# I2-Multimedia-Lab/Video-Frame-Interpolation-Based-on-Deformable-Kernel-Region

Hardware: AMD Instinct MI355X
Metric: interpolated frames/sec at 1080p (hot path only: correlation + DepthFlowProjection + FilterInterpolation of DAIN_slowmotion x4) (higher is better)
Workload: dtype f32

## Files before the change

### video-frame-interpolation-based-on-deformable-kernel-region_amd/csrc/filterinterp_lds.hip

```cpp
#include "filterinterp_dev.h"
#include "filterinterp_paths.h"

namespace vfi {

#define FI_TW 64
#define FI_TH 16
#define FI_PX 2
#define FI_THREADS (FI_TW * FI_TH / FI_PX)
#define FI_PASS_ROWS (FI_TH / FI_PX)
#define FI_KS (FI_PX / 2)
#define FI_HDR 16
#define FI_RING_FLOATS 20464
#define FI_RMAX 5
#define FI_WAVES (8 / FI_PX)
#define FI_KTOP (15 * FI_KS)
static_assert(2 * FI_KTOP * FI_THREADS <= FI_RING_FLOATS, "the largest window takes two ring slots");
#define FI_B64_MIN_BH 34
#define FI_B64_MIN_BW 92
#define FI_B64_PITCH_SKEW 32

struct FiPixel {
    bool valid, inimg;
    float alpha, beta;
    int lbase;
    bool odd;
    unsigned pix;
    float f[16];
};
#define FI_BLEND_MAXC 4
struct FiBlend { const float* other; float* out; float w0, w2; };

template <int K, bool BLEND>
__device__ __forceinline__ void fi_run_channels(const float* __restrict__ img, float* __restrict__ out, int64_t cs,
                                                int c_begin, int c_end, int tid, const FiWindow& win,
                                                const FiPixel (&px)[FI_PX], float* __restrict__ ring, const FiBlend& bl) {
    constexpr int R = (FI_RING_FLOATS / (K * FI_THREADS)) < FI_RMAX ? (FI_RING_FLOATS / (K * FI_THREADS)) : FI_RMAX;
    static_assert(R >= 2 && (R - 2) * K <= 63, "vmcnt is a 6-bit counter");
    const float inv_pitch32 = 1.0f / (float)win.pitch;
    unsigned goff[K];
#pragma unroll
    for (int k = 0; k < K; ++k) {
        const int e = tid + k * FI_THREADS;
        const int r = fi_row_of(e, inv_pitch32);
        const int col = e - r * win.pitch;
        const unsigned off = 4u * (unsigned)(clampi(win.by0 + r, 0, win.h - 1) * win.hs + clampi(win.bx0 + col, 0, win.w - 1));
        goff[k] = (col < win.bw && r < win.bh) ? off : 0x80000000u;
    }
    const int plane_bytes = 4 * ((win.h - 1) * win.hs + win.w);
    constexpr int NP = K * FI_THREADS;
    constexpr int D = R - 1;
    auto issue = [&](int c, int slot) {
        const auto plane = buffer_rsrc(img + (int64_t)c * cs, plane_bytes);
        float* l = ring + slot * NP + tid;
#pragma unroll
        for (int k = 0; k < K; ++k)
            __builtin_amdgcn_raw_ptr_buffer_load_lds(plane, (lds_ptr_t)(l + k * FI_THREADS), 4, goff[k], 0, 0, 0);
    };
    auto finish = [&](int c, int p, const float (&v)[16], float* o) {
        const float val = fi4_pixel(v, px[p].f, px[p].alpha, px[p].beta);
        o[px[p].pix] = val;
        if constexpr (BLEND) {
            const float* bi = bl.other + (int64_t)c * cs;
            const float q0 = bi[px[p].pix] * bl.w0, q2 = val * bl.w2;
            float* bo = bl.out + (int64_t)c * cs;
            bo[px[p].pix] = q0 + q2;
        }
    };
    auto compute = [&](int c, int slot) {
        float* o = out + (int64_t)c * cs;
        const float* base = ring + slot * NP;
        {
#pragma unroll
            for (int p = 0; p < FI_PX; ++p) {
                if (px[p].valid) {
                    const float* t = base + px[p].lbase;
                    float v[16];
#pragma unroll
                    for (int r = 0; r < 4; ++r)
#pragma unroll
                        for (int k = 0; k < 4; ++k) v[r * 4 + k] = t[r * win.pitch + k];
                    finish(c, p, v, o);
                }
            }
        }
    };

    if (c_begin >= c_end) return;
    const int last = c_end - 1;
    for (int j = 0; j < D; ++j)
        if (c_begin + j <= last) issue(c_begin + j, j);
    wait_windows<K>(min(c_begin + D - 1, last) - c_begin);
    __builtin_amdgcn_s_barrier();
    int slot = 0;
    for (int c = c_begin; c <= last; ++c) {
        if (c + D <= last) issue(c + D, slot == 0 ? R - 1 : slot - 1);
        compute(c, slot);
        if (c < last) wait_windows<K>(min(c + D, last) - (c + 1));
        __builtin_amdgcn_s_barrier();
        slot = (slot + 1 == R) ? 0 : slot + 1;
    }
#pragma unroll
    for (int p = 0; p < FI_PX; ++p)
        if (px[p].inimg && !px[p].valid)
            for (int c = c_begin; c < c_end; ++c) {
                const float val = img[(int64_t)c * cs + px[p].pix];
                out[(int64_t)c * cs + px[p].pix] = val;
                if constexpr (BLEND) {
                    const float q0 = bl.other[(int64_t)c * cs + px[p].pix] * bl.w0, q2 = val * bl.w2;
                    bl.out[(int64_t)c * cs + px[p].pix] = q0 + q2;
                }
            }
}

template <int K, bool B64, bool DMA16 = false>
__device__ __forceinline__ void fi_run_channels_lean(const float* __restrict__ img, float* __restrict__ out, int64_t cs,
                                                     int c_begin, int c_end, int tid, const FiWindow& win,
                                                     const FiPixel (&px)[FI_PX], float* __restrict__ ring) {
    typedef float v2f __attribute__((ext_vector_type(2)));
    constexpr int EPT = DMA16 ? 4 : 1;
    constexpr int NP = K * FI_THREADS * EPT;
    constexpr int R = (FI_RING_FLOATS / NP) < FI_RMAX ? (FI_RING_FLOATS / NP) : FI_RMAX;
    constexpr int D = R - 1;
    static_assert(D >= 1 && (D - 1) * K <= 63, "ring geometry");
    static_assert((FI_HDR * 4) % 8 == 0 && (NP * 4) % 8 == 0 && FI_B64_PITCH_SKEW % 2 == 0, "8-byte tap reads stay 8-byte aligned");
    if (c_begin >= c_end) return;
    const float inv_pitch32 = 1.0f / (float)win.pitch;
    unsigned goff[K];
#pragma unroll
    for (int k = 0; k < K; ++k) {
        const int e = (tid + k * FI_THREADS) * EPT;
        const int r = fi_row_of(e, inv_pitch32);
        const int col = e - r * win.pitch;
        const unsigned off = 4u * (unsigned)(clampi(win.by0 + r, 0, win.h - 1) * win.hs + (DMA16 ? win.bx0 + col : clampi(win.bx0 + col, 0, win.w - 1)));
        goff[k] = (col < win.bw && r < win.bh) ? off : 0x80000000u;
    }
    const int plane_bytes = 4 * ((win.h - 1) * win.hs + win.w);
    const int wave_first = __builtin_amdgcn_readfirstlane(tid >> 6) * 64;
    const unsigned ring_lds = (unsigned)(uintptr_t)(lds_ptr_t)ring;
    const unsigned pitch4 = 4u * (unsigned)win.pitch;
    unsigned lb[FI_PX], soff[FI_PX];
#pragma unroll
    for (int p = 0; p < FI_PX; ++p) {
        lb[p] = ring_lds + 4u * (unsigned)px[p].lbase;
        soff[p] = px[p].valid ? 4u * px[p].pix : 0x80000000u;
    }
    v2f F[FI_PX][8];
#pragma unroll
    for (int p = 0; p < FI_PX; ++p)
#pragma unroll
        for (int r = 0; r < 4; ++r) {
            F[p][2 * r] = v2f{px[p].f[4 * r], px[p].f[4 * r + 2]};
            F[p][2 * r + 1] = v2f{px[p].f[4 * r + 1], px[p].f[4 * r + 3]};
        }
    const int last = c_end - 1;
    const float* pdma = img + (int64_t)c_begin * cs;
    float* pout = out + (int64_t)c_begin * cs;
    constexpr bool ONE = DMA16;
    auto din = buffer_rsrc(pdma, 0x7fffffff);
    auto dout = buffer_rsrc(pout, 0x7fffffff);
    const int cs4 = (int)(cs * 4);
    const int soff_max = 0x7fffffff - plane_bytes - cs4;
    int sin = 0, sout = 0;
    auto next_in = [&]() {
        if (__builtin_expect(sin > soff_max, 0)) {
            asm volatile("; the input descriptor moves up" ::: "memory");
            pdma = (const float*)((const char*)pdma + sin);
            din = buffer_rsrc(pdma, 0x7fffffff);
            sin = 0;
        }
        sin += cs4;
    };
    auto next_out = [&]() {
        if (__builtin_expect(sout > soff_max, 0)) {
            asm volatile("; the output descriptor moves up" ::: "memory");
            pout = (float*)((char*)pout + sout);
            dout = buffer_rsrc(pout, 0x7fffffff);
            sout = 0;
        }
        sout += cs4;
    };
    constexpr unsigned SLOT = NP * 4, RING = R * SLOT;
    auto issue = [&](unsigned slot) {
        const auto plane = buffer_rsrc(pdma, plane_bytes);
        float* l = ring + (slot >> 2) + wave_first * EPT;
#pragma unroll
        for (int k = 0; k < K; ++k) {
            if constexpr (ONE) __builtin_amdgcn_raw_ptr_buffer_load_lds(din, (lds_ptr_t)(l + k * FI_THREADS * EPT), 4 * EPT, goff[k], sin, 0, 0);
            else __builtin_amdgcn_raw_ptr_buffer_load_lds(plane, (lds_ptr_t)(l + k * FI_THREADS * EPT), 4 * EPT, goff[k], 0, 0, 0);
        }
        if constexpr (ONE) { next_in(); return; }
        pdma += cs;
    };
#define FI_READ2(dst, addr, o0, o1) asm volatile("ds_read2_b32 %0, %1 offset0:" #o0 " offset1:" #o1 : "=v"(dst) : "v"(addr))
#define FI_READ64(dst, addr, o) asm volatile("ds_read_b64 %0, %1 offset:" #o : "=v"(dst) : "v"(addr))
    auto compute = [&](unsigned so) {
        const auto oplane = buffer_rsrc(pout, plane_bytes);
        constexpr int NQ = B64 ? 12 : 8;
        constexpr int PART0 = B64 ? 3 : 4;
        v2f q[2][NQ];
        auto reads = [&q, &lb, so, pitch4](auto P, auto H) {
            constexpr int p = decltype(P)::value, h = decltype(H)::value;
            v2f (&d)[NQ] = q[p & 1];
            if constexpr (B64) {
                if constexpr (h == 0) {
                    const unsigned a = lb[p] + so;
                    FI_READ64(d[0], a, 0); FI_READ64(d[1], a, 8); FI_READ64(d[2], a, 16);
                } else {
                    unsigned a = lb[p] + so;
#pragma unroll
                    for (int r = 1; r < 4; ++r) { a += pitch4; FI_READ64(d[3 * r], a, 0); FI_READ64(d[3 * r + 1], a, 8); FI_READ64(d[3 * r + 2], a, 16); }
                }
            } else {
                unsigned a = lb[p] + so + (h ? 2u * pitch4 : 0u);
                FI_READ2(d[4 * h], a, 0, 2); FI_READ2(d[4 * h + 1], a, 1, 3);
                a += pitch4;
                FI_READ2(d[4 * h + 2], a, 0, 2); FI_READ2(d[4 * h + 3], a, 1, 3);
            }
        };
        auto arrived = [&](auto P) {
            constexpr int p = decltype(P)::value;
            constexpr int later = (p + 1 < FI_PX) ? PART0 : 0;
            v2f (&d)[NQ] = q[p & 1];
            if constexpr (B64)
                asm volatile("s_waitcnt lgkmcnt(%12)" : "+v"(d[0]), "+v"(d[1]), "+v"(d[2]), "+v"(d[3]), "+v"(d[4]), "+v"(d[5]),
                                                         "+v"(d[6]), "+v"(d[7]), "+v"(d[8]), "+v"(d[9]), "+v"(d[10]), "+v"(d[11]) : "n"(later));
            else
                asm volatile("s_waitcnt lgkmcnt(%8)" : "+v"(d[0]), "+v"(d[1]), "+v"(d[2]), "+v"(d[3]), "+v"(d[4]), "+v"(d[5]),
                                                        "+v"(d[6]), "+v"(d[7]) : "n"(later));
        };
        auto pixel = [&](auto P) {
            constexpr int p = decltype(P)::value;
            const v2f (&d)[NQ] = q[p & 1];
            float val;
            if constexpr (B64) {
                const bool odd = px[p].odd;
                float v[16];
#pragma unroll
                for (int r = 0; r < 4; ++r) {
                    v[r * 4 + 0] = odd ? d[3 * r].y : d[3 * r].x;
                    v[r * 4 + 1] = odd ? d[3 * r + 1].x : d[3 * r].y;
                    v[r * 4 + 2] = odd ? d[3 * r + 1].y : d[3 * r + 1].x;
                    v[r * 4 + 3] = odd ? d[3 * r + 2].x : d[3 * r + 1].y;
                }
                val = fi4_pixel(v, px[p].f, px[p].alpha, px[p].beta);
            } else {
                v2f top = d[0] * F[p][0];
                top = __builtin_elementwise_fma(d[1], F[p][1], top);
                top = __builtin_elementwise_fma(d[2], F[p][2], top);
                top = __builtin_elementwise_fma(d[3], F[p][3], top);
                v2f bot = d[4] * F[p][4];
                bot = __builtin_elementwise_fma(d[5], F[p][5], bot);
                bot = __builtin_elementwise_fma(d[6], F[p][6], bot);
                bot = __builtin_elementwise_fma(d[7], F[p][7], bot);
                val = blend4(px[p].alpha, px[p].beta, top.x, top.y, bot.x, bot.y);
            }
            if constexpr (ONE) __builtin_amdgcn_raw_buffer_store_b32(__float_as_uint(val), dout, soff[p], sout, 0);
            else __builtin_amdgcn_raw_buffer_store_b32(__float_as_uint(val), oplane, soff[p], 0, 0);
        };
        using I0 = std::integral_constant<int, 0>;
        using I1 = std::integral_constant<int, 1>;
        reads(I0{}, I0{}); reads(I0{}, I1{});
        if constexpr (FI_PX > 1) reads(I1{}, I0{});
        static_for<0, FI_PX>([&](auto P) {
            constexpr int p = decltype(P)::value;
            arrived(P);
            pixel(P);
            if constexpr (p + 1 < FI_PX) reads(std::integral_constant<int, p + 1>{}, I1{});
            if constexpr (p + 2 < FI_PX) reads(std::integral_constant<int, p + 2>{}, I0{});
        });
        if constexpr (ONE) { next_out(); return; }
        pout += cs;
    };
    constexpr bool SKEW = !B64 && FI_PX == 2 && K <= 7 * FI_KS;
    constexpr int NQS = B64 ? 12 : 8;
    v2f qa[NQS], qb[NQS];
    auto rd_all = [&](v2f (&d)[NQS], int p, unsigned so) {
        unsigned a = lb[p] + so;
#pragma unroll
        for (int r = 0; r < 4; ++r) {
            if constexpr (B64) { FI_READ64(d[3 * r], a, 0); FI_READ64(d[3 * r + 1], a, 8); FI_READ64(d[3 * r + 2], a, 16); }
            else { FI_READ2(d[2 * r], a, 0, 2); FI_READ2(d[2 * r + 1], a, 1, 3); }
            a += pitch4;
        }
    };
    auto arrived_s = [&](v2f (&d)[NQS], auto LATER) {
        constexpr int later = decltype(LATER)::value;
        if constexpr (B64)
            asm volatile("s_waitcnt lgkmcnt(%12)" : "+v"(d[0]), "+v"(d[1]), "+v"(d[2]), "+v"(d[3]), "+v"(d[4]), "+v"(d[5]),
                                                     "+v"(d[6]), "+v"(d[7]), "+v"(d[8]), "+v"(d[9]), "+v"(d[10]), "+v"(d[11]) : "n"(later));
        else
            asm volatile("s_waitcnt lgkmcnt(%8)" : "+v"(d[0]), "+v"(d[1]), "+v"(d[2]), "+v"(d[3]), "+v"(d[4]), "+v"(d[5]),
                                                    "+v"(d[6]), "+v"(d[7]) : "n"(later));
    };
    auto fma_store = [&](const v2f (&d)[NQS], int p, const float* plane_ptr) {
        float val;
        if constexpr (B64) {
            const bool odd = px[p].odd;
            float v[16];
#pragma unroll
            for (int r = 0; r < 4; ++r) {
                v[r * 4 + 0] = odd ? d[3 * r].y : d[3 * r].x;
                v[r * 4 + 1] = odd ? d[3 * r + 1].x : d[3 * r].y;
                v[r * 4 + 2] = odd ? d[3 * r + 1].y : d[3 * r + 1].x;
                v[r * 4 + 3] = odd ? d[3 * r + 2].x : d[3 * r + 1].y;
            }
            val = fi4_pixel(v, px[p].f, px[p].alpha, px[p].beta);
        } else {
            v2f top = d[0] * F[p][0];
            top = __builtin_elementwise_fma(d[1], F[p][1], top);
            top = __builtin_elementwise_fma(d[2], F[p][2], top);
            top = __builtin_elementwise_fma(d[3], F[p][3], top);
            v2f bot = d[4] * F[p][4];
            bot = __builtin_elementwise_fma(d[5], F[p][5], bot);
            bot = __builtin_elementwise_fma(d[6], F[p][6], bot);
            bot = __builtin_elementwise_fma(d[7], F[p][7], bot);
            val = blend4(px[p].alpha, px[p].beta, top.x, top.y, bot.x, bot.y);
        }
        if constexpr (ONE) {
            __builtin_amdgcn_raw_buffer_store_b32(__float_as_uint(val), dout, soff[p], sout - (p ? cs4 : 0), 0);
        } else {
            const auto oplane = buffer_rsrc(plane_ptr, plane_bytes);
            __builtin_amdgcn_raw_buffer_store_b32(__float_as_uint(val), oplane, soff[p], 0, 0);
        }
    };
    auto compute_skewed = [&](unsigned so, bool first) {
        rd_all(qa, 0, so);
        if (!first) fma_store(qb, 1, pout - cs);
        if constexpr (B64) asm volatile("s_waitcnt lgkmcnt(3)" ::: "memory"); else asm volatile("s_waitcnt lgkmcnt(7)" ::: "memory");
        rd_all(qb, 1, so);
        arrived_s(qa, std::integral_constant<int, NQS>{});
        fma_store(qa, 0, pout);
        arrived_s(qb, std::integral_constant<int, 0>{});
        if constexpr (ONE) { next_out(); return; }
        pout += cs;
    };
    const int n0 = min(D, c_end - c_begin);
    for (int j = 0; j < n0; ++j) issue((unsigned)j * SLOT);
    wait_windows<K>(n0 - 1);
    __builtin_amdgcn_s_barrier();
    int c = c_begin;
    unsigned slot = 0, freed = RING - SLOT;
    if constexpr (SKEW) {
        for (; c + D <= last; ++c) {
            issue(freed);
            compute_skewed(slot, c == c_begin);
            asm volatile("s_waitcnt vmcnt(%0)" ::"n"((D - 1) * K) : "memory");
            __builtin_amdgcn_s_barrier();
            freed = slot; slot = (slot + SLOT == RING) ? 0u : slot + SLOT;
        }
        for (; c <= last; ++c) {
            compute_skewed(slot, c == c_begin);
            if (c < last) {
                asm volatile("s_waitcnt vmcnt(0)" ::: "memory");
                __builtin_amdgcn_s_barrier();
            }
            freed = slot; slot = (slot + SLOT == RING) ? 0u : slot + SLOT;
        }
        fma_store(qb, 1, pout - cs);
    }
    for (; c + D <= last; ++c) {
        issue(freed);
        compute(slot);
        asm volatile("s_waitcnt vmcnt(%0)" ::"n"((D - 1) * K) : "memory");
        __builtin_amdgcn_s_barrier();
        freed = slot; slot = (slot + SLOT == RING) ? 0u : slot + SLOT;
    }
    for (; c <= last; ++c) {
        compute(slot);
        if (c < last) {
            asm volatile("s_waitcnt vmcnt(0)" ::: "memory");
            __builtin_amdgcn_s_barrier();
        }
        freed = slot; slot = (slot + SLOT == RING) ? 0u : slot + SLOT;
    }
#undef FI_READ2
#undef FI_READ64
#pragma unroll
    for (int p = 0; p < FI_PX; ++p)
        if (px[p].inimg && !px[p].valid)
            for (int cc = c_begin; cc < c_end; ++cc) out[(int64_t)cc * cs + px[p].pix] = img[(int64_t)cc * cs + px[p].pix];
}

template <bool BLEND>
__global__ __launch_bounds__(FI_THREADS, FI_WAVES) void fi_forward_ori_lds(
    const float* __restrict__ in1, const float* __restrict__ in2, const float* __restrict__ in3,
    float* __restrict__ out, int channel, int h, int w,
    vfi_strides s1, vfi_strides s2, vfi_strides s3,
    int tiles_x, int tiles_y, int ntiles, int ch_per_group, int aligned16, FiBlend blend) {
    __shared__ __attribute__((aligned(16))) float lds[FI_HDR + FI_RING_FLOATS];

    const int tile = fi_xcd_tile<int>(blockIdx.x);
    if (tile >= ntiles) return;
    const FiTile tp = fi_tile_at(tile, tiles_x, tiles_y, channel, ch_per_group);
    const int b = tp.b, c_begin = tp.c_begin, c_end = tp.c_end;

    const int tid = threadIdx.x;
    const int x = tp.tx * FI_TW + (tid & (FI_TW - 1));
    const int y0 = tp.ty * FI_TH + (tid >> 6);

    FiPixel px[FI_PX];
    int L[FI_PX], T[FI_PX];
    int bx_lo = INT_MAX, by_lo = INT_MAX, bx_hi = INT_MIN, by_hi = INT_MIN;
    float fxv[FI_PX], fyv[FI_PX];
#pragma unroll
    for (int p = 0; p < FI_PX; ++p) {
        const int y = y0 + p * FI_PASS_ROWS;
        px[p].inimg = x < w && y < h;
        px[p].pix = (unsigned)(y * (int)s1.h + x);
        fxv[p] = fyv[p] = 0.0f;
#pragma unroll
        for (int k = 0; k < 16; ++k) px[p].f[k] = 0.0f;
        if (px[p].inimg) {
            const float* flow = in2 + (int64_t)b * s2.b + (int64_t)y * s2.h + x;
            fxv[p] = flow[0];
            fyv[p] = flow[s2.c];
            const float* fpx = in3 + (int64_t)b * s3.b + (int64_t)y * s3.h + x;
#pragma unroll
            for (int k = 0; k < 16; ++k) px[p].f[k] = fpx[(int64_t)k * s3.c];
        }
    }
#pragma unroll
    for (int p = 0; p < FI_PX; ++p) {
        const int y = y0 + p * FI_PASS_ROWS;
        const float fx = fxv[p], fy = fyv[p];
        const float x2 = (float)x + fx;
        const float y2 = (float)y + fy;
        px[p].valid = px[p].inimg && fi_valid(fx, fy, x2, y2, w, h);
        const int ix = px[p].valid ? (int)x2 : 0, iy = px[p].valid ? (int)y2 : 0;
        L[p] = ix - 1;
        T[p] = iy - 1;
        px[p].alpha = x2 - (float)ix;
        px[p].beta = y2 - (float)iy;
        if (px[p].valid) {
            bx_lo = min(bx_lo, L[p]); by_lo = min(by_lo, T[p]);
            bx_hi = max(bx_hi, L[p] + 3); by_hi = max(by_hi, T[p] + 3);
        }
    }

    int* box = reinterpret_cast<int*>(lds);
    if (tid == 0) fi_box_clear(box);
    __syncthreads();
    const bool any_valid = fi_box_fold(box, tid, bx_lo, by_lo, bx_hi, by_hi);
    const int raw_bh = any_valid ? box[3] - box[1] + 1 : 0;
    const int raw_bw = any_valid ? box[2] - box[0] + 1 : 0;
    constexpr bool lean = !BLEND;
    const bool can16 = lean && aligned16 && any_valid && box[0] >= 0 && box[2] < w;
    const int lo = can16 ? (box[0] & ~3) : box[0];
    const int bw64 = any_valid ? box[2] - (lo & ~1) + 1 : 0;
    const bool fits64 = ((((bw64 + 31) >> 6) << 6) + FI_B64_PITCH_SKEW) * raw_bh <= 10 * FI_KS * FI_THREADS;
    const bool use64 = lean && fits64 && (raw_bh >= FI_B64_MIN_BH || raw_bw >= FI_B64_MIN_BW);
    const int bx0 = (use64 && any_valid) ? (lo & ~1) : lo, by0 = box[1];
    const int bw = any_valid ? box[2] - bx0 + 1 : 0;
    const int bh = raw_bh;
    const int pitch = use64 ? (((bw + 31) >> 6) << 6) + FI_B64_PITCH_SKEW : fi_pitch_for(bw);
    const int n = pitch * bh;

#pragma unroll
    for (int p = 0; p < FI_PX; ++p) {
        const int lc = L[p] - bx0;
        px[p].odd = use64 && (lc & 1);
        px[p].lbase = (T[p] - by0) * pitch + (use64 ? (lc & ~1) : lc);
    }

    const float* img = in1 + (int64_t)b * s1.b;
    float* dst = out + (int64_t)b * s1.b;
    const FiBlend bl{blend.other ? blend.other + (int64_t)b * s1.b : nullptr, blend.out ? blend.out + (int64_t)b * s1.b : nullptr,
                     blend.w0, blend.w2};

    const int kmax = (n + FI_THREADS - 1) / FI_THREADS;
    if (kmax > FI_KTOP) {
#pragma unroll
        for (int p = 0; p < FI_PX; ++p) {
            if (px[p].valid) {
                fi4_channels_direct(img, dst + px[p].pix, c_begin, c_end, s1.c, (int)s1.h, h, w, L[p], T[p], px[p].f,
                                    px[p].alpha, px[p].beta);
            } else if (px[p].inimg) {
                for (int c = c_begin; c < c_end; ++c) dst[(int64_t)c * s1.c + px[p].pix] = img[(int64_t)c * s1.c + px[p].pix];
            }
            if (BLEND && px[p].inimg)
                for (int c = c_begin; c < c_end; ++c) {
                    const float q0 = bl.other[(int64_t)c * s1.c + px[p].pix] * bl.w0, q2 = dst[(int64_t)c * s1.c + px[p].pix] * bl.w2;
                    bl.out[(int64_t)c * s1.c + px[p].pix] = q0 + q2;
                }
        }
        return;
    }

    const FiWindow win{bx0, by0, bw, bh, pitch, h, w, (int)s1.h};
    float* ring = lds + FI_HDR;
#define FI_RUN(K) if constexpr (lean) { \
        if constexpr ((K) <= 10 * FI_KS) { if (use64) fi_run_channels_lean<K, true>(img, dst, s1.c, c_begin, c_end, tid, win, px, ring); } \
        if (!use64) fi_run_channels_lean<K, false>(img, dst, s1.c, c_begin, c_end, tid, win, px, ring); \
    } else fi_run_channels<K, BLEND>(img, dst, s1.c, c_begin, c_end, tid, win, px, ring, bl)
    if constexpr (lean) {
        const int k16 = (n + 4 * FI_THREADS - 1) / (4 * FI_THREADS);
        if (can16 && k16 <= 3) {
#define FI_RUN16(K) { if (use64) fi_run_channels_lean<K, true, true>(img, dst, s1.c, c_begin, c_end, tid, win, px, ring); \
                      else fi_run_channels_lean<K, false, true>(img, dst, s1.c, c_begin, c_end, tid, win, px, ring); }
            if (k16 <= 1) FI_RUN16(1) else if (k16 == 2) FI_RUN16(2) else FI_RUN16(3)
#undef FI_RUN16
            return;
        }
    }
    if (kmax <= 2 * FI_KS) FI_RUN(2 * FI_KS);
    else if (kmax <= 3 * FI_KS) FI_RUN(3 * FI_KS);
    else if (kmax <= 4 * FI_KS) FI_RUN(4 * FI_KS);
    else if (kmax <= 5 * FI_KS) FI_RUN(5 * FI_KS);
    else if (kmax <= 6 * FI_KS) FI_RUN(6 * FI_KS);
    else if (kmax <= 7 * FI_KS) FI_RUN(7 * FI_KS);
    else if (kmax <= 8 * FI_KS) FI_RUN(8 * FI_KS);
    else if (kmax <= 10 * FI_KS) FI_RUN(10 * FI_KS);
    else if (kmax <= 12 * FI_KS) FI_RUN(12 * FI_KS);
    else FI_RUN(15 * FI_KS);
#undef FI_RUN
}

template __global__ void fi_forward_ori_lds<true>(const float* __restrict__, const float* __restrict__, const float* __restrict__,
    float* __restrict__, int, int, int, vfi_strides, vfi_strides, vfi_strides, int, int, int, int, int, FiBlend);
template __global__ void fi_forward_ori_lds<false>(const float* __restrict__, const float* __restrict__, const float* __restrict__,
    float* __restrict__, int, int, int, vfi_strides, vfi_strides, vfi_strides, int, int, int, int, int, FiBlend);

}

using namespace vfi;

static int forward_ori_lds(const float* input1, const float* input2, const float* input3, float* output, int batch, int channel,
                           int h, int w, vfi_strides s1, vfi_strides s2, vfi_strides s3, vfi_stream_t stream, FiBlend blend) {
    if ((int64_t)h * s1.h * 4 > INT_MAX) return FI_DECLINED;
    const int tiles_x = (w + FI_TW - 1) / FI_TW, tiles_y = (h + FI_TH - 1) / FI_TH;
    const int64_t nt = (int64_t)tiles_x * tiles_y * batch;
    if (nt > (1 << 28)) return FI_DECLINED;
    const int ntiles = (int)nt;

    const FiSplit split = blend.out ? FiSplit{channel, 1} : fi_channel_split(ntiles, channel, 4.3);

    const dim3 grid((unsigned)fi_xcd_grid<8>(ntiles), (unsigned)split.groups, 1);
    const int aligned16 = !(w & 3) && !(s1.h & 3) && !(s1.c & 3) && !(s1.b & 3) && !((uintptr_t)input1 & 15) &&
                          s1.c > 0 && 4 * s1.c + 4 * ((int64_t)(h - 1) * s1.h + w) < 0x7fffffffLL;
    if (blend.out)
        hipLaunchKernelGGL(fi_forward_ori_lds<true>, grid, dim3(FI_THREADS, 1, 1), 0, (hipStream_t)stream, input1, input2,
                           input3, output, channel, h, w, s1, s2, s3, tiles_x, tiles_y, ntiles, split.ch_per_group, aligned16, blend);
    else
        hipLaunchKernelGGL(fi_forward_ori_lds<false>, grid, dim3(FI_THREADS, 1, 1), 0, (hipStream_t)stream, input1, input2,
                           input3, output, channel, h, w, s1, s2, s3, tiles_x, tiles_y, ntiles, split.ch_per_group, aligned16, blend);
    return launch_status();
}

int vfi::launch_fi_ori_lds(const float* input1, const float* input2, const float* input3, float* output, int batch, int channel,
                           int h, int w, vfi_strides s1, vfi_strides s2, vfi_strides s3, vfi_stream_t stream) {
    return forward_ori_lds(input1, input2, input3, output, batch, channel, h, w, s1, s2, s3, stream, FiBlend{nullptr, nullptr, 0.0f, 0.0f});
}

int vfi::launch_fi_ori_lds_blend(const float* input1, const float* input2, const float* input3, float* output, const float* other,
                                 float* blend, float w0, float w2, int batch, int channel, int h, int w, vfi_strides s1,
                                 vfi_strides s2, vfi_strides s3, vfi_stream_t stream) {
    if (channel > FI_BLEND_MAXC || !other || !blend) return FI_DECLINED;
    return forward_ori_lds(input1, input2, input3, output, batch, channel, h, w, s1, s2, s3, stream, FiBlend{other, blend, w0, w2});
}
```

Measured before the change: 436.9.

## Add channel-interleaved LDS path for FilterInterpolation with packed FMA math

Adds a new FilterInterpolation inner routine that stages 2 or 4 channels per ring slot, interleaved in LDS, so each pixel reads a vector per tap. The 4x4 filter and bilinear weights are applied with packed v_pk_fma_f32 instructions, and staging of the next slot is double-buffered against the compute. The lean kernel path takes this route when the tile window fits a slot and there are enough channels. The channel split is also rounded up to multiples of 4. This trades more LDS per element and a noinline call for fewer LDS reads and ALU ops per channel, though the changed channel grouping may unbalance work.

Result: slower. 334.6 (-23.4%).

```diff
diff --git a/video-frame-interpolation-based-on-deformable-kernel-region_amd/csrc/filterinterp_il.h b/video-frame-interpolation-based-on-deformable-kernel-region_amd/csrc/filterinterp_il.h
--- /dev/null
+++ b/video-frame-interpolation-based-on-deformable-kernel-region_amd/csrc/filterinterp_il.h
@@ -0,0 +1,163 @@
+#pragma once
+
+namespace vfi {
+
+typedef float fi_v2f __attribute__((ext_vector_type(2)));
+template <int HI>
+__device__ __forceinline__ fi_v2f fi_pk_mul_sel(fi_v2f d, fi_v2f f) {
+    fi_v2f o;
+    if constexpr (HI) asm("v_pk_mul_f32 %0, %1, %2 op_sel:[0,1]" : "=v"(o) : "v"(d), "v"(f));
+    else asm("v_pk_mul_f32 %0, %1, %2 op_sel_hi:[1,0]" : "=v"(o) : "v"(d), "v"(f));
+    return o;
+}
+template <int HI>
+__device__ __forceinline__ fi_v2f fi_pk_fma_sel(fi_v2f d, fi_v2f f, fi_v2f acc) {
+    fi_v2f o;
+    if constexpr (HI) asm("v_pk_fma_f32 %0, %1, %2, %3 op_sel:[0,1,0]" : "=v"(o) : "v"(d), "v"(f), "v"(acc));
+    else asm("v_pk_fma_f32 %0, %1, %2, %3 op_sel_hi:[1,0,1]" : "=v"(o) : "v"(d), "v"(f), "v"(acc));
+    return o;
+}
+
+template <int M, int K>
+__device__ __noinline__
+void fi_run_channels_il(const float* __restrict__ img_, float* __restrict__ out_, int64_t cs_, int c_begin_, int c_end_, int tid,
+                        const FiWindow& win_, const FiPixel (&px)[FI_PX], float* __restrict__ ring_) {
+    static_assert(M == 4 || M == 2, "channels per ring step");
+    auto uni = [](int v) { return __builtin_amdgcn_readfirstlane(v); };
+    auto uni64 = [&](uint64_t v) { return ((uint64_t)(unsigned)uni((int)(v >> 32)) << 32) | (unsigned)uni((int)v); };
+    const float* __restrict__ img = (const float*)uni64((uint64_t)img_);
+    float* __restrict__ out = (float*)uni64((uint64_t)out_);
+    const int64_t cs = (int64_t)uni64((uint64_t)cs_);
+    const int c_begin = uni(c_begin_), c_end = uni(c_end_);
+    const FiWindow win{uni(win_.bx0), uni(win_.by0), uni(win_.bw), uni(win_.bh), uni(win_.pitch), uni(win_.h), uni(win_.w), uni(win_.hs)};
+    float* ring = (float*)uni64((uint64_t)ring_);
+    typedef float vt __attribute__((ext_vector_type(M)));
+    typedef __attribute__((address_space(3))) char* lds_bytes_t;
+    typedef __attribute__((address_space(3))) vt* lds_vt_t;
+    constexpr unsigned EB = 4u * M;
+    constexpr unsigned SLOT = FI_IL_SLOT_BYTES;
+    static_assert(SLOT % 16 == 0 && 2 * SLOT <= 4u * FI_RING_FLOATS && (FI_HDR * 4) % 16 == 0, "two 16-byte aligned slots");
+    static_assert((unsigned)K * FI_THREADS * EB < SLOT + FI_THREADS * EB, "K is the smallest count that covers a slot");
+    if (c_begin >= c_end) return;
+
+    const float inv_pitch = 1.0f / (float)win.pitch;
+    unsigned goff[K];
+#pragma unroll
+    for (int k = 0; k < K; ++k) {
+        const int e = tid + k * FI_THREADS;
+        const int r = fi_row_of(e, inv_pitch);
+        const int col = e - r * win.pitch;
+        const unsigned off = 4u * (unsigned)(clampi(win.by0 + r, 0, win.h - 1) * win.hs + clampi(win.bx0 + col, 0, win.w - 1));
+        goff[k] = (col < win.bw && r < win.bh) ? off : 0x80000000u;
+    }
+    const int plane_bytes = 4 * ((win.h - 1) * win.hs + win.w);
+    const lds_bytes_t lring = (lds_bytes_t)ring;
+    const lds_bytes_t lmine = lring + (unsigned)tid * EB;
+    const unsigned pitch_b = EB * (unsigned)win.pitch;
+    unsigned lb[FI_PX], soff[FI_PX];
+    fi_v2f F[FI_PX][8], W[FI_PX][2];
+#pragma unroll
+    for (int p = 0; p < FI_PX; ++p) {
+        lb[p] = px[p].valid ? EB * (unsigned)px[p].lbase : 0u;
+        soff[p] = px[p].valid ? 4u * px[p].pix : 0x80000000u;
+        const float a = px[p].alpha, b = px[p].beta;
+        W[p][0] = fi_v2f{(1.0f - a) * (1.0f - b), a * (1.0f - b)};
+        W[p][1] = fi_v2f{(1.0f - a) * b, a * b};
+#pragma unroll
+        for (int i = 0; i < 8; ++i) F[p][i] = fi_v2f{px[p].f[2 * i], px[p].f[2 * i + 1]};
+    }
+
+    auto load = [&](int c, const float* plane0, vt (&pf)[K]) {
+        const float* pl = plane0;
+#pragma unroll
+        for (int j = 0; j < M; ++j) {
+            const auto plane = buffer_rsrc(pl, c + j < c_end ? plane_bytes : 0);
+#pragma unroll
+            for (int k = 0; k < K; ++k)
+                pf[k][j] = __uint_as_float(__builtin_amdgcn_raw_buffer_load_b32(plane, goff[k], 0, 0));
+            pl += cs;
+        }
+    };
+    auto stage = [&](unsigned so, const vt (&pf)[K]) {
+#pragma unroll
+        for (int k = 0; k < K; ++k) {
+            if ((unsigned)(k + 1) * FI_THREADS * EB <= SLOT)
+                *(lds_vt_t)(lmine + so + (unsigned)k * FI_THREADS * EB) = pf[k];
+            else
+                *(lds_vt_t)(lring + so + min((unsigned)(tid + k * FI_THREADS) * EB, SLOT - EB)) = pf[k];
+        }
+    };
+    auto pixel = [&](auto P, int c, float* oplane0, unsigned so) {
+        constexpr int p = decltype(P)::value;
+        constexpr int H = M / 2;
+        const lds_bytes_t t = lring + so + lb[p];
+        fi_v2f q[4][H];
+        static_for<0, 4>([&](auto R) {
+            constexpr int r = decltype(R)::value;
+            const lds_vt_t row = (lds_vt_t)(t + r * pitch_b);
+            const vt d[4] = {row[0], row[1], row[2], row[3]};
+            constexpr int l = r & 2, rr = (r & 2) + 1;
+            static_for<0, H>([&](auto HH) {
+                constexpr int hh = decltype(HH)::value;
+                fi_v2f d0, d1, d2, d3;
+                if constexpr (M == 4) {
+                    if constexpr (hh == 0) { d0 = d[0].xy; d1 = d[1].xy; d2 = d[2].xy; d3 = d[3].xy; }
+                    else { d0 = d[0].zw; d1 = d[1].zw; d2 = d[2].zw; d3 = d[3].zw; }
+                } else { d0 = d[0]; d1 = d[1]; d2 = d[2]; d3 = d[3]; }
+                if constexpr (r & 1) {
+                    q[l][hh] = fi_pk_fma_sel<0>(d0, F[p][2 * r], q[l][hh]);
+                    q[rr][hh] = fi_pk_fma_sel<0>(d2, F[p][2 * r + 1], q[rr][hh]);
+                } else {
+                    q[l][hh] = fi_pk_mul_sel<0>(d0, F[p][2 * r]);
+                    q[rr][hh] = fi_pk_mul_sel<0>(d2, F[p][2 * r + 1]);
+                }
+                q[l][hh] = fi_pk_fma_sel<1>(d1, F[p][2 * r], q[l][hh]);
+                q[rr][hh] = fi_pk_fma_sel<1>(d3, F[p][2 * r + 1], q[rr][hh]);
+            });
+        });
+        float v[M];
+        static_for<0, H>([&](auto HH) {
+            constexpr int hh = decltype(HH)::value;
+            fi_v2f t2 = fi_pk_mul_sel<0>(q[0][hh], W[p][0]);
+            t2 = fi_pk_fma_sel<1>(q[1][hh], W[p][0], t2);
+            t2 = fi_pk_fma_sel<0>(q[2][hh], W[p][1], t2);
+            t2 = fi_pk_fma_sel<1>(q[3][hh], W[p][1], t2);
+            v[2 * hh] = t2.x;
+            v[2 * hh + 1] = t2.y;
+        });
+        float* pl = oplane0;
+#pragma unroll
+        for (int j = 0; j < M; ++j) {
+            const auto oplane = buffer_rsrc(pl, c + j < c_end ? plane_bytes : 0);
+            __builtin_amdgcn_raw_buffer_store_b32(__float_as_uint(v[j]), oplane, soff[p], 0, 0);
+            pl += cs;
+        }
+    };
+
+    vt pf[K];
+    const float* pin = img + (int64_t)c_begin * cs;
+    float* pout = out + (int64_t)c_begin * cs;
+    load(c_begin, pin, pf);
+    stage(0u, pf);
+    __builtin_amdgcn_fence(__ATOMIC_RELEASE, "workgroup");
+    __builtin_amdgcn_s_barrier();
+    unsigned so = 0;
+    for (int c = c_begin; c < c_end; c += M) {
+        pin += (int64_t)M * cs;
+        load(c + M, pin, pf);
+        static_for<0, FI_PX>([&](auto P) {
+            pixel(P, c, pout, so);
+            if constexpr (decltype(P)::value == FI_IL_STAGE_AFTER_PIXEL) stage(SLOT - so, pf);
+        });
+        __builtin_amdgcn_fence(__ATOMIC_RELEASE, "workgroup");
+        __builtin_amdgcn_s_barrier();
+        so = SLOT - so;
+        pout += (int64_t)M * cs;
+    }
+#pragma unroll
+    for (int p = 0; p < FI_PX; ++p)
+        if (px[p].inimg && !px[p].valid)
+            for (int cc = c_begin; cc < c_end; ++cc) out[(int64_t)cc * cs + px[p].pix] = img[(int64_t)cc * cs + px[p].pix];
+}
+
+}
diff --git a/video-frame-interpolation-based-on-deformable-kernel-region_amd/csrc/filterinterp_lds.hip b/video-frame-interpolation-based-on-deformable-kernel-region_amd/csrc/filterinterp_lds.hip
--- a/video-frame-interpolation-based-on-deformable-kernel-region_amd/csrc/filterinterp_lds.hip
+++ b/video-frame-interpolation-based-on-deformable-kernel-region_amd/csrc/filterinterp_lds.hip
@@ -18,6 +18,13 @@
 #define FI_B64_MIN_BH 34
 #define FI_B64_MIN_BW 92
 #define FI_B64_PITCH_SKEW 32
+#define FI_IL_MINC 8
+#define FI_IL_SLOT_BYTES (FI_RING_FLOATS * 4 / 2 / 16 * 16)
+#define FI_IL_PITCH4 16
+#define FI_IL_PITCH2 32
+#ifndef FI_IL_STAGE_AFTER_PIXEL
+#define FI_IL_STAGE_AFTER_PIXEL 0
+#endif
 
 struct FiPixel {
     bool valid, inimg;
@@ -29,6 +36,10 @@
 };
 #define FI_BLEND_MAXC 4
 struct FiBlend { const float* other; float* out; float w0, w2; };
+
+}
+#include "filterinterp_il.h"
+namespace vfi {
 
 template <int K, bool BLEND>
 __device__ __forceinline__ void fi_run_channels(const float* __restrict__ img, float* __restrict__ out, int64_t cs,
@@ -464,6 +475,31 @@
 
     const float* img = in1 + (int64_t)b * s1.b;
     float* dst = out + (int64_t)b * s1.b;
+
+    if constexpr (lean) {
+        const int il_p4 = (raw_bw + FI_IL_PITCH4 - 1) & ~(FI_IL_PITCH4 - 1), il_p2 = (raw_bw + FI_IL_PITCH2 - 1) & ~(FI_IL_PITCH2 - 1);
+        const int il_m = (!any_valid || c_end - c_begin < FI_IL_MINC) ? 0
+                         : il_p4 * raw_bh * 16 < FI_IL_SLOT_BYTES ? 4 : il_p2 * raw_bh * 8 < FI_IL_SLOT_BYTES ? 2 : 0;
+        if (il_m) {
+            const int il_pitch = il_m == 4 ? il_p4 : il_p2;
+            const FiWindow il_win{box[0], by0, raw_bw, raw_bh, il_pitch, h, w, (int)s1.h};
+            FiPixel il_px[FI_PX];
+#pragma unroll
+            for (int p = 0; p < FI_PX; ++p) {
+                il_px[p] = px[p];
+                il_px[p].lbase = (T[p] - by0) * il_pitch + (L[p] - box[0]);
+            }
+            const int kil = (il_pitch * raw_bh + FI_THREADS - 1) / FI_THREADS;
+#define FI_RUN_IL(M, K) fi_run_channels_il<M, K>(img, dst, s1.c, c_begin, c_end, tid, il_win, il_px, lds + FI_HDR)
+            if (il_m == 4) {
+                if (kil <= 3) FI_RUN_IL(4, 3); else if (kil == 4) FI_RUN_IL(4, 4); else FI_RUN_IL(4, 5);
+            } else {
+                if (kil <= 6) FI_RUN_IL(2, 6); else if (kil <= 8) FI_RUN_IL(2, 8); else FI_RUN_IL(2, 10);
+            }
+#undef FI_RUN_IL
+            return;
+        }
+    }
     const FiBlend bl{blend.other ? blend.other + (int64_t)b * s1.b : nullptr, blend.out ? blend.out + (int64_t)b * s1.b : nullptr,
                      blend.w0, blend.w2};
 
@@ -532,7 +568,11 @@
     if (nt > (1 << 28)) return FI_DECLINED;
     const int ntiles = (int)nt;
 
-    const FiSplit split = blend.out ? FiSplit{channel, 1} : fi_channel_split(ntiles, channel, 4.3);
+    FiSplit split = blend.out ? FiSplit{channel, 1} : fi_channel_split(ntiles, channel, 4.3);
+    if (!blend.out && split.groups > 1 && split.ch_per_group >= FI_IL_MINC) {
+        split.ch_per_group = (split.ch_per_group + 3) & ~3;
+        split.groups = (channel + split.ch_per_group - 1) / split.ch_per_group;
+    }
 
     const dim3 grid((unsigned)fi_xcd_grid<8>(ntiles), (unsigned)split.groups, 1);
     const int aligned16 = !(w & 3) && !(s1.h & 3) && !(s1.c & 3) && !(s1.b & 3) && !((uintptr_t)input1 & 15) &&
```
